# leggedrobotics/open3d_slam_private

Measured on AMD Instinct MI355X. Metric: ICP iterations/sec (scan-to-map), higher is better.
Workload: dtype f32

## Files before the change

### open3d_slam_private_amd/capi.py

```python
from __future__ import annotations

import ctypes as C
import math
import os
import subprocess

import numpy as np

_HERE = os.path.dirname(os.path.abspath(__file__))
_SO = os.environ.get("O3D_REG_LIB") or os.path.join(_HERE, "lib", "libo3dslam_reg.so")

STATUS_NAMES = {0: "OK", 1: "EMPTY_TARGET", 2: "EMPTY_SOURCE", 3: "NO_CORRESPONDENCES", 4: "BAD_TRANSFORM",
                5: "NOT_CONFIGURED", 6: "BAD_ARGUMENT", 7: "MISSING_FIELD", 8: "DEVICE_ERROR", 9: "UNSUPPORTED",
                10: "OUT_OF_BOUNDS"}
OUT_OF_BOUNDS = 10
COST_P2PL, COST_GICP = 0, 1
COST_O3D_P2PL, COST_O3D_P2P = 2, 3
SMOOTH_LEN_MAX = 15


class RegError(RuntimeError):
    def __init__(self, status, msg=""):
        self.status = status
        super().__init__(f"{STATUS_NAMES.get(status, status)}: {msg}")
# ... 1359 lines not shown
    lib = load_library()
    s = np.ascontiguousarray(sums, np.float64)
    To = np.zeros(16, np.float32)
    rank = C.c_int32()
    st = lib.reg_solve_update(C.byref(params), _ptr(s), _ptr(_T_in(T_iter)), _ptr(To), C.byref(rank))
    if st != 0:
        raise RegError(st, "reg_solve_update")
    return _T_out(To), rank.value


def host_solve6(A, b):
    x = np.zeros(6, np.float32)
    rank = load_library().reg_host_solve6(_ptr(_f32(A).reshape(36)), _ptr(_f32(b)), _ptr(x))
    return x, rank


def host_solve6_xicp(A, b, flags):
    x = np.zeros(6, np.float32)
    f = np.ascontiguousarray(flags, np.int32)
    rank = load_library().reg_host_solve6_xicp(_ptr(_f32(A).reshape(36)), _ptr(_f32(b)), _ptr(f), _ptr(x))
    return x, rank


def host_x_to_T(x):
    T = np.zeros(16, np.float32)
    load_library().reg_host_x_to_T(_ptr(_f32(x)), _ptr(T))
    return _T_out(T)


def host_centroid(xyz):
    xyz = _f32(xyz)
    out = np.zeros(3, np.float32)
    load_library().reg_host_centroid(_ptr(xyz), xyz.shape[1], xyz.shape[0], _ptr(out))
    return out


def host_o3d_update(cost, sums):
    s = np.ascontiguousarray(sums, np.float64).reshape(32)
    U = np.zeros(16, np.float64)
    rank = C.c_int32()
    st = load_library().reg_host_o3d_update(int(cost), _ptr(s), _ptr(U), C.byref(rank))
    if st != 0:
        raise RegError(st, "reg_host_o3d_update")
    return U.reshape(4, 4).T.copy(), rank.value


def host_tail_plan(n, cus=256, tile=0):
    lib = load_library()
    lib.reg_host_tail_plan.argtypes = [C.c_int64, C.c_int32, C.c_int32, C.POINTER(C.c_int32)]
    lib.reg_host_tail_plan.restype = None
    out = (C.c_int32 * 4)()
    lib.reg_host_tail_plan(int(n), int(cus), int(tile), out)
    return bool(out[0]), int(out[1]), int(out[2]), int(out[3])
```

### open3d_slam_private_amd/csrc/host_loop.hpp

```cpp
#pragma once


static reg_status check_ready(reg_handle* h, bool need_prepared) {
    if (!h) return REG_BAD_ARGUMENT;
    if (!h->device_ok) return REG_DEVICE_ERROR;
    if (h->m == 0) {
        h->err = "no reference set (reg_set_target)";
        return REG_NOT_CONFIGURED;
    }
    if (h->n == 0) {
        h->err = "no reading set (reg_set_source)";
        return REG_NOT_CONFIGURED;
    }
    if (need_prepared && !h->prepared) {
        h->err = "reg_prepare has not been called for this reading";
        return REG_NOT_CONFIGURED;
    }
    return REG_OK;
}

static reg_status prepare_rowmajor(reg_handle* h, const float* T_init_row, const float* c_override = nullptr,
                                   int64_t n_global = 0, const IterState* init_state = nullptr) {
    reg_status s = check_ready(h, false);
    if (s != REG_OK) return s;
// ... 44 lines not shown
        si.init = *init_state;
        si.dst = h->i_iter.as<IterState>();
    } else {
        std::memset(&si.init, 0, sizeof(si.init));
    }
    k_prepare_source<<<grid_for(n), 256, 0, h->stream>>>(
        h->s_raw.as<float>(), h->s_stride, (p2pl && h->has_snrm) ? h->s_nrm_raw.as<float>() : nullptr, h->s_nstride, n, pa,
        p2pl ? 1 : 0, h->perm, h->s_xyz.as<float4>(), (p2pl && h->has_snrm) ? h->s_nrm.as<float4>() : nullptr,
        h->i_hint.as<uint8_t>(), h->i_hist.as<uint32_t>(), h->i_acc.as<double>(), kAccRows * kSums, si,
        h->i_cache.as<float4>());
    if (h->prm.cost == REG_COST_GICP)
        k_pack_cov<<<grid_for(n), 256, 0, h->stream>>>(h->s_cov_raw.as<float>(), n, h->perm, h->s_cov.as<float4>());
    pmark("prepare_source");
    HIPCHK(h, hipGetLastError());
    h->prepared = true;
    h->match_launches = 0;
    h->have_match = false;
    h->pm_have_match = false;
    return REG_OK;
}


static void xicp_frame_change(const reg_handle* h, float Trd12[12]) {
    float A[16], Trd[16];
    m4_identity(A);
    for (int k = 0; k < 3; ++k) A[4 * k + 3] = -h->c_ref[k];
    m4_mul(A, h->T_init, Trd);
    for (int k = 0; k < 12; ++k) Trd12[k] = Trd[k];
}

static reg_status build_iter_state(reg_handle* h, const float* T_row, int update, IterState* st) {
    std::memset(st, 0, sizeof(IterState));
    for (int i = 0; i < 16; ++i) {
        st->T[i] = T_row[i];
        st->Td[i] = (double)T_row[i];
    }
    st->chk = Checkers();
    st->chk.max_iter = h->prm.max_iter;
    st->chk.min_diff_rot = h->prm.min_diff_rot;
    st->chk.min_diff_trans = h->prm.min_diff_trans;
    st->chk.smooth_len = h->prm.smooth_len;
    st->chk.init(T_row);
    st->cost = h->prm.cost;
    st->fixed_iters = h->prm.fixed_iters;
    st->max_iter = h->prm.max_iter;
    st->update = update;
    st->gicp_rot_eps = h->prm.gicp_rot_eps;
    st->gicp_trans_eps = h->prm.gicp_trans_eps;
    st->gicp_stop_rule = h->prm.gicp_stop_rule;
    st->gicp_rel_fitness = h->prm.gicp_rel_fitness;
    st->gicp_rel_rmse = h->prm.gicp_rel_rmse;
    st->n_total = (float)(h->n_total_hint > 0 ? h->n_total_hint : h->n);
    st->band_lo = st->band_hi = INFINITY;
    st->limit_last = st->limit_prev = INFINITY;
    st->use_trim = (h->prm.cost == REG_COST_P2PL && h->prm.use_trimmed) ? 1 : 0;
    st->trim_ratio = h->prm.trim_ratio;
    st->band_cap = kBandCap;
    st->qcount = h->i_qcount.as<unsigned int>();
    st->debug_narrow_band = ((h->dbg.debug_flags & 8) ? 1 : 0) | ((h->dbg.debug_flags & 64) ? 2 : 0);
    h->xicp_pending = false;
    for (int k = 0; k < 6; ++k) st->xicp_flags[k] = 1;
    if (h->prm.use_xicp && h->prm.cost == REG_COST_P2PL && update) {
        HIPCHK(h, h->i_xicp.reserve(sizeof(XicpState)));
        st->xicp_stage = 1;
        st->xicp_enough = h->prm.xicp_enough;
        st->xicp_insufficient = h->prm.xicp_insufficient;
        st->xicp_cos_min = (float)std::cos((double)h->prm.xicp_min_angle_deg * 3.14159265358979323846 / 180.0);
        st->xicp_cos_strong = (float)std::cos((double)h->prm.xicp_strong_angle_deg * 3.14159265358979323846 / 180.0);
        xicp_frame_change(h, st->xicp_Trd);
        h->xicp_pending = true;
    }
    return REG_OK;
}

static reg_status init_iter_state(reg_handle* h, const float* T_row, int update) {
    IterState* st = h->h_iter;
    if (h->iter_copy_pending) HIPCHK(h, hipEventSynchronize(h->ev_iter));
    reg_status s = build_iter_state(h, T_row, update, st);
    if (s != REG_OK) return s;
    HIPCHK(h, hipMemcpyAsync(h->i_iter.p, st, sizeof(IterState), hipMemcpyHostToDevice, h->stream));
    HIPCHK(h, hipEventRecord(h->ev_iter, h->stream));
    h->iter_copy_pending = true;
    return REG_OK;
}

static reg_status enqueue_match(reg_handle* h, bool zero_hist = false) {
    const bool trim = h->prm.cost == REG_COST_P2PL && h->prm.use_trimmed;
    if (trim && zero_hist) HIPCHK(h, hipMemsetAsync(h->i_hist.p, 0, 3 * 2048 * 4, h->stream));
    const bool fused_hist = h->dbg.match_variant == 3;
    uint32_t* hist0 = (trim && fused_hist) ? h->i_hist.as<uint32_t>() : nullptr;
    uint32_t* hist2 = trim ? h->i_hist.as<uint32_t>() + 4096 : nullptr;
    const IterState* it = h->i_iter.as<IterState>();
    if (h->dbg.match_variant == 1) {
        prof_mark(h, 0, true);
        k_match<<<h->n_blocks, 256, 0, h->stream>>>(h->s_xyz.as<float4>(), h->n, it, h->grid, h->i_pos.as<int>(),
                                                    h->i_d2.as<float>(), hist0, hist2, h->shift0);
        prof_mark(h, 0, false);
    } else {
        uint8_t* hint = h->dbg.match_variant == 2 ? nullptr : h->i_hint.as<uint8_t>();
        const int lanes = h->dbg.lanes_per_point == 4 ? 4 : (h->dbg.lanes_per_point == 2 ? 2 : 8);
        const int blocks = grid_for(h->n * lanes);
        const int tile = h->match_launches < 2 ? h->env.xcd_tile_first : h->env.xcd_tile_later;
        ++h->match_launches;
        const dim3 grid(xcd_tiled_grid(blocks, tile)), block(256);
        auto go = [&](auto kernel) {
            launch_timed(h, 0, kernel, grid, block, 0, (const float4*)h->s_xyz.as<float4>(), h->n, it, h->grid,
                         h->i_pos.as<int>(), h->i_d2.as<float>(), hist0, hist2, hint, h->shift0, h->dbg.debug_flags, blocks,
// ... 441 lines not shown
    if (h->env.hints) {
        std::vector<uint8_t> hv((size_t)h->n);
        if (hipMemcpy(hv.data(), h->i_hint.p, (size_t)h->n, hipMemcpyDeviceToHost) == hipSuccess) {
            long long cnt[18] = {0};
            for (uint8_t v : hv) ++cnt[v < 17 ? v : 17];
            fprintf(stderr, "[o3dreg] terminating level of the last iteration (halo, then levels with rho =");
            for (int l = 0; l < h->grid.n_levels; ++l) fprintf(stderr, " %.3f", h->grid.rho[l]);
            fprintf(stderr, "):");
            for (int l = 0; l <= h->grid.n_levels; ++l) fprintf(stderr, " %lld", cnt[l]);
            fprintf(stderr, "\n");
        }
    }
    if (h->env.coh_stats) {
        CohStats cs;
        if (hipMemcpy(&cs, h->i_stats.p, sizeof(cs), hipMemcpyDeviceToHost) == hipSuccess) {
            fprintf(stderr, "[o3dreg] coherent fused iterations: %llu point-iterations, %llu searched (%.2f %%)\n", cs.n_points,
                    cs.n_searched, cs.n_points ? 100.0 * (double)cs.n_searched / (double)cs.n_points : 0.0);
            (void)hipMemset(h->i_stats.p, 0, sizeof(cs));
        }
    }
    if (h->env.stamps) {
        fprintf(stderr, "update kernel stamps (cycles): reduce %llu [rows %llu select %llu band-add %llu] solve %llu update+check %llu mirror %llu\n", mir->stamps[0],
                mir->stamps[4], mir->stamps[5], mir->stamps[6], mir->stamps[1], mir->stamps[2], mir->stamps[3]);
        fprintf(stderr, "   select detail: verify+stage-issue %llu, zero+hist+barriers %llu, wave0 pick/rank %llu\n", mir->stamps[3], mir->stamps[7] >> 32, mir->stamps[7] & 0xffffffffull);
    }
    if (h->profiling) {
        for (size_t i = 0; i + 1 < h->prof_ev.size(); i += 2) {
            float ms = 0;
            if (hipEventElapsedTime(&ms, h->prof_ev[i], h->prof_ev[i + 1]) == hipSuccess) {
                const int kind = h->prof_kind[i / 2];
                res->prof_ms[kind] += ms;
                res->prof_launches[kind] += 1;
            }
        }
        for (hipEvent_t e : h->prof_ev) (void)hipEventDestroy(e);
        h->prof_ev.clear();
        h->prof_kind.clear();
        h->profiling = false;
    }
}

static reg_status register_pm(reg_handle* h, const float* Ti, float T_out[16], reg_result* res);

extern "C" {

void reg_host_tail_plan(int64_t n, int32_t cus, int32_t tile, int32_t plan[4]) {
    const TailPlan pl = tail_plan_for(n, cus, 0, tile);
    plan[0] = pl.ok ? 1 : 0;
    plan[1] = pl.grid;
    plan[2] = pl.wpc;
    plan[3] = pl.chunk8;
}

reg_status reg_prepare(reg_handle* h, const float T_init[16]) {
    if (!h || !T_init) return REG_BAD_ARGUMENT;
    float Tr[16];
    col_to_row(T_init, Tr);
    return prepare_rowmajor(h, Tr);
}

reg_status reg_linearize(reg_handle* h, const float T_iter[16], float H[36], float b[6], double* err,
                         int64_t* n_inliers) {
    reg_status s = check_ready(h, true);
    if (s != REG_OK) return s;
    if (!T_iter) return REG_BAD_ARGUMENT;
    if (h->prm.cost == REG_COST_O3D_P2P) {
        h->err = "reg_linearize: point-to-point (Umeyama) has no normal equations";
        return REG_UNSUPPORTED;
    }
    if (h->pm_on) {
        h->err = "reg_linearize: not available with a libpointmatcher chain (reg_set_pm_chain)";
        return REG_UNSUPPORTED;
    }
    float Tr[16];
    col_to_row(T_iter, Tr);
    if (!m4_is_finite(Tr)) return REG_BAD_TRANSFORM;
    HIPCHK(h, hipSetDevice(h->prm.device));
    s = iterate_once(h, Tr, true);
    if (s != REG_OK) return s;
    const double* sums = h->h_mirror->sums;
    if (H && b) sums_to_system(sums, h->prm.cost, H, b);
    if (err) *err = sums[27];
    if (n_inliers) *n_inliers = (int64_t)llround(sums[28]);
    if (sums[28] == 0.0) {
        h->err = "ErrorMinimizer: no point to minimize";
        return REG_NO_CORRESPONDENCES;
    }
    return REG_OK;
}

reg_status reg_register(reg_handle* h, const float T_init[16], float T_out[16], reg_result* res) {
    if (!h || !T_init || !T_out) return REG_BAD_ARGUMENT;
    reg_result local;
    if (!res) res = &local;
    std::memset(res, 0, sizeof(*res));
    std::memcpy(T_out, T_init, 64);
    float Ti[16];
    col_to_row(T_init, Ti);
    const auto t_reg0 = std::chrono::steady_clock::now();
    auto rmark = [&](const char* what) {
        if (h->env.trace)
            fprintf(stderr, "[o3dreg] register %-14s t=%.1fus\n", what,
                    std::chrono::duration<double, std::micro>(std::chrono::steady_clock::now() - t_reg0).count());
    };
    if (h->pm_on) return register_pm(h, Ti, T_out, res);
    const bool p2pl = h->prm.cost == REG_COST_P2PL;
// ... 199 lines not shown
```

### open3d_slam_private_amd/csrc/kernels_tail.hpp

```cpp
#pragma once

#ifndef O3D_TAIL_ACQ
#define O3D_TAIL_ACQ 0
#endif
#ifndef O3D_TAIL_THREADS
#define O3D_TAIL_THREADS 512
#endif
constexpr int kTailThreads = O3D_TAIL_THREADS;
#ifndef O3D_TAIL_SLOTS
#define O3D_TAIL_SLOTS 1024
#endif
#ifndef O3D_TAIL_WGS_PER_CU
#define O3D_TAIL_WGS_PER_CU 1
#endif
constexpr int kTailSlots = O3D_TAIL_SLOTS;
constexpr int kTailWgsPerCu = O3D_TAIL_WGS_PER_CU;
constexpr int kTailPts = kTailSlots / kTailThreads;
constexpr int kTailBandCap = 1024;
constexpr int kTailRec = 12;
constexpr int kTailHistRow = 32;
constexpr int kTailCoarse = 256;
constexpr float kTailWideRel = 0.02f;
constexpr int kTailMaxIters = 64;
constexpr int kTailSyncWords = 256;
constexpr int kTailRing = 4;
constexpr int kTailBandCntWord = 128;
constexpr int kTailAccRows = 16;
constexpr int kTailAccDoubles = kTailRing * kTailAccRows * kSums;
constexpr int kTailSyncBytes = kTailSyncWords * 4 + kTailAccDoubles * 8;
constexpr int kTailArriveStride = 16;
constexpr int kTailErrWord = 192;
constexpr int kTailSearchedWord = 193;
constexpr int kTailItersWord = 194;
constexpr int kTailCauseWord = 195;
constexpr int kTailStampWord = 200;
constexpr int kTailGroups = kTailThreads / 8;
constexpr int kTailBins = 1024;
#ifndef O3D_TAIL_STAMPS
#define O3D_TAIL_STAMPS 0
#endif
#ifndef O3D_TAIL_G4
#define O3D_TAIL_G4 0
#endif
#if O3D_TAIL_STAMPS
#define TAIL_STAMP(i)                                                      \
    do {                                                                   \
        const unsigned long long now_ = __builtin_amdgcn_s_memrealtime();  \
        stamp_acc[i] += now_ - stamp_last;                                 \
        stamp_last = now_;                                                 \
    } while (0)
#else
#define TAIL_STAMP(i) do { } while (0)
#endif

struct TailCfg {
    int64_t n;
    int chunk8;
    int wpc;
    int tile;
    int max_iters;
    float slack;
    unsigned long long seq;
    unsigned long long timeout_ticks;
};

struct TailLds {
    static constexpr int kRows = 0;
    static constexpr int kUnion = kRows + 5 * kTailSlots * 16;
    static constexpr int kUnionSeg = (kTailThreads / 8) * kSegWords<8> * 4, kUnionSeg4 = O3D_TAIL_G4 ? (kTailThreads / 4) * kSegWords<4> * 4 : 0;
    static constexpr int kUnionMax = kUnionSeg > kUnionSeg4 ? (kUnionSeg > kTailBandCap * 8 ? kUnionSeg : kTailBandCap * 8)
                                                            : (kUnionSeg4 > kTailBandCap * 8 ? kUnionSeg4 : kTailBandCap * 8);
    static constexpr int kUnionBytes = (kUnionMax + 255) & ~255;
    static constexpr int kD2 = kUnion + kUnionBytes;
    static constexpr int kFail = kD2 + kTailSlots * 4;
    static constexpr int kWcls = kFail + kTailSlots * 2;
    static constexpr int kHint = kWcls + kTailSlots;
    static constexpr int kSh = kHint + kTailSlots;
    static constexpr int kTot = kSh + 16 * kSums * 8;
    static constexpr int kState = kTot + kSums * 8;
    static constexpr int kStateBytes = (int)((sizeof(IterState) + 15) & ~size_t(15));
    static constexpr int kMisc = kState + kStateBytes;
    static constexpr int kWtot = kMisc + 64;
    static constexpr int kOff = kWtot + 64;
    static constexpr int kX = kOff + 272 * 4;
    static constexpr int kMirror = kX + 96;
    static constexpr int kMirrorBytes = (int)((sizeof(HostMirror) + 15) & ~size_t(15));
    static constexpr int kHist = kMirror + kMirrorBytes;
    static constexpr int kTotal = kHist + kTailBins * 4;
    static constexpr int kBk = kUnion;
};
static_assert(TailLds::kBk + kTailBandCap * 8 - TailLds::kUnion <= TailLds::kUnionBytes, "phase-C scratch exceeds the union");
static_assert(kTailGroups * kSegWords<8> * 4 <= TailLds::kUnionBytes, "segment lists exceed the union");
static_assert(TailLds::kTotal * kTailWgsPerCu <= 160 * 1024, "LDS budget of one CU");
constexpr int kTailLdsBytes = TailLds::kTotal;

__device__ __forceinline__ double tail_ld_f64(const double* p) {
    const unsigned long long v = __hip_atomic_load(reinterpret_cast<unsigned long long*>(const_cast<double*>(p)), __ATOMIC_RELAXED,
                                                   __HIP_MEMORY_SCOPE_AGENT);
    return __longlong_as_double((long long)v);
}
__device__ __forceinline__ void tail_st_f64(double* p, double x) {
    __hip_atomic_store(reinterpret_cast<unsigned long long*>(p), (unsigned long long)__double_as_longlong(x), __ATOMIC_RELAXED,
                       __HIP_MEMORY_SCOPE_AGENT);
}
__device__ __forceinline__ unsigned long long tail_ld_u64(const void* p) {
    return __hip_atomic_load(reinterpret_cast<unsigned long long*>(const_cast<void*>(p)), __ATOMIC_RELAXED, __HIP_MEMORY_SCOPE_AGENT);
}
__device__ __forceinline__ void tail_st_u64(void* p, unsigned long long x) {
    __hip_atomic_store(reinterpret_cast<unsigned long long*>(p), x, __ATOMIC_RELAXED, __HIP_MEMORY_SCOPE_AGENT);
}
__device__ __forceinline__ unsigned tail_ld_u32(const unsigned* p) {
    return __hip_atomic_load(const_cast<unsigned*>(p), __ATOMIC_RELAXED, __HIP_MEMORY_SCOPE_AGENT);
}

__device__ __noinline__ void tail_solve_update(IterState* sit, const double* tot, const uint32_t* misc, float* s_x, bool trim,
                                               unsigned n_band_raw) {
    const int lane = (int)(threadIdx.x & 63);
    const float r_limit_last = sit->limit_last, r_limit_sel = __uint_as_float(misc[2]);
    const int r_dbg_narrow = sit->debug_narrow_band & 1;
    const int r_fixed = sit->fixed_iters, r_iters = sit->iterations;
    const int r_xnc = sit->xicp_nc;
    const double r_tot28 = tot[28];
    float r_T[16];
#pragma unroll
    for (int i = 0; i < 16; ++i) r_T[i] = sit->T[i];
    const int r = lane >> 3, c = lane & 7;
    double a = 0.0;
    if (r < 6 && c < 7) {
        if (c < 6) {
            const int lo = r < c ? r : c, hi = r < c ? c : r;
            const int k = lo * 6 - (lo * (lo - 1)) / 2 + (hi - lo);
            a = (double)(float)tot[k];
        } else {
            a = (double)(-(float)tot[21 + r]);
        }
    }
    const double a_orig = a;
    double dmax = 0.0;
#pragma unroll
    for (int j = 0; j < 6; ++j) dmax = fmax(dmax, fabs(__shfl(a_orig, j * 8 + j)));
    bool well = dmax > 0.0;
    const double piv_thr = 1e-4 * dmax;
#pragma unroll
    for (int j = 0; j < 6; ++j) {
        const double pj = __shfl(a, j * 8 + j);
        well = well && (pj > piv_thr);
        const double ajc = __shfl(a, j * 8 + c);
        const double arj = __shfl(a, r * 8 + j);
        const double qd = ajc / pj;
        a = (r == j) ? qd : a - arj * qd;
    }
    double xsol[6];
#pragma unroll
    for (int i = 0; i < 6; ++i) xsol[i] = __shfl(a, i * 8 + 6);
    if (lane != 0) return;
    const float limit = r_limit_sel;
    sit->limit_prev = r_limit_last;
    sit->limit_last = limit;
    if (!trim || !(limit < INFINITY)) {
        sit->band_lo = INFINITY;
        sit->band_hi = INFINITY;
    } else {
        const float prev = r_limit_last;
        float m = 0.3f;
        if (prev < INFINITY && prev > 0.f) m = fminf(fmaxf(2.0f * fabsf(limit - prev) / limit + 0.003f, 0.003f), 0.6f);
        if (r_dbg_narrow) m = 1e-7f;
        sit->band_lo = limit * (1.0f - m);
        sit->band_hi = limit * (1.0f + m);
    }
    sit->band_count = n_band_raw;
    sit->stall = 0;
    if (r_tot28 == 0.0) {
        sit->status = REG_NO_CORRESPONDENCES;
        sit->done = 1;
        return;
    }
    float x[6], dT[16], Tn[16];
    int rank = 6;
    if (r_xnc > 0) {
        rank = upd_solve6_xicp(tot, sit->xicp_flags, s_x);
        for (int i = 0; i < 6; ++i) x[i] = s_x[i];
    } else if (well) {
        for (int i = 0; i < 6; ++i) x[i] = (float)xsol[i];
    } else {
        rank = upd_solve6_p2pl(tot, s_x);
        for (int i = 0; i < 6; ++i) x[i] = s_x[i];
    }
    sit->rank_last = rank;
    x_to_T(x, dT);
    m4_mul(dT, r_T, Tn);
    for (int i = 0; i < 16; ++i) sit->T_prev[i] = r_T[i];
    for (int i = 0; i < 16; ++i) sit->T[i] = Tn[i];
    sit->iterations = r_iters + 1;
    bool iterate;
    if (r_fixed > 0)
        iterate = r_iters + 1 < r_fixed;
    else
        iterate = sit->chk.check(Tn);
    if (!iterate) sit->done = 1;
}

__device__ __forceinline__ void tail_gicp_factor(const Xf& T, const float4 s, const float4 a0, const float4 a1, const float4 q,
                                                 const float4 b0, const float4 b1, float d2, double (&v)[kSums]) {
    const float3 tp = xf_point(T, s.x, s.y, s.z);
    const double r[3] = {(double)q.x - (double)tp.x, (double)q.y - (double)tp.y, (double)q.z - (double)tp.z};
    const double Cp[9] = {a0.x, a0.y, a0.z, a0.y, a0.w, a1.x, a0.z, a1.x, a1.y};
    const double Cq[9] = {b0.x, b0.y, b0.z, b0.y, b0.w, b1.x, b0.z, b1.x, b1.y};
    double R[9];
#pragma unroll
    for (int a = 0; a < 3; ++a)
#pragma unroll
        for (int c = 0; c < 3; ++c) R[3 * a + c] = (double)T.m[4 * a + c];
    double RC[9], S[9];
#pragma unroll
    for (int a = 0; a < 3; ++a)
#pragma unroll
        for (int c = 0; c < 3; ++c) {
            double t = 0;
#pragma unroll
            for (int k = 0; k < 3; ++k) t += R[3 * a + k] * Cp[3 * k + c];
            RC[3 * a + c] = t;
// ... 44 lines not shown
        }
        Mr[a] = Mi[3 * a] * r[0] + Mi[3 * a + 1] * r[1] + Mi[3 * a + 2] * r[2];
    }
    int k = 0;
#pragma unroll
    for (int a = 0; a < 6; ++a)
#pragma unroll
        for (int c = a; c < 6; ++c) {
            double t = 0;
#pragma unroll
            for (int kk = 0; kk < 3; ++kk) t += J[6 * kk + a] * MJ[6 * kk + c];
            v[k++] += t;
        }
#pragma unroll
    for (int a = 0; a < 6; ++a) v[21 + a] += J[a] * Mr[0] + J[6 + a] * Mr[1] + J[12 + a] * Mr[2];
    v[27] += 0.5 * (r[0] * Mr[0] + r[1] * Mr[1] + r[2] * Mr[2]);
    v[28] += 1.0;
    v[29] += 1.0;
    v[30] += (double)d2;
}

__device__ __noinline__ void tail_solve_update_gicp(IterState* sit, const double* tot, double* s_dl) {
    const int lane = (int)(threadIdx.x & 63);
    const int r = lane >> 3, c = lane & 7;
    double a = 0.0;
    if (r < 6 && c < 7) {
        if (c < 6) {
            const int lo = r < c ? r : c, hi = r < c ? c : r;
            a = tot[lo * 6 - (lo * (lo - 1)) / 2 + (hi - lo)];
        } else {
            a = -tot[21 + r];
        }
    }
    const double a_orig = a;
    double dmax = 0.0;
#pragma unroll
    for (int j = 0; j < 6; ++j) dmax = fmax(dmax, fabs(__shfl(a_orig, j * 8 + j)));
    bool well = dmax > 0.0;
    const double piv_thr = 1e-10 * dmax;
#pragma unroll
    for (int j = 0; j < 6; ++j) {
        const double pj = __shfl(a, j * 8 + j);
        well = well && (pj > piv_thr);
        const double ajc = __shfl(a, j * 8 + c);
        const double arj = __shfl(a, r * 8 + j);
        const double qd = ajc / pj;
        a = (r == j) ? qd : a - arj * qd;
    }
    double xsol[6];
#pragma unroll
    for (int i = 0; i < 6; ++i) xsol[i] = __shfl(a, i * 8 + 6);
    if (lane != 0) return;
    const double cnt = tot[28];
    sit->limit_prev = sit->limit_last;
    sit->limit_last = INFINITY;
    sit->band_lo = INFINITY;
    sit->band_hi = INFINITY;
    sit->band_count = 0;
    sit->stall = 0;
    float r_T[16];
    for (int i = 0; i < 16; ++i) r_T[i] = sit->T[i];
    if (cnt == 0.0) {
        sit->status = REG_NO_CORRESPONDENCES;
        sit->done = 1;
        return;
    }
    const double fit = cnt / (double)sit->n_total, rmse = sqrt(tot[30] / cnt);
    if (sit->gicp_stop_rule == 1 && sit->fixed_iters <= 0) {
        const bool conv = sit->iterations >= 1 && fabs(fit - sit->fit_prev) < (double)sit->gicp_rel_fitness &&
                          fabs(rmse - sit->rmse_prev) < (double)sit->gicp_rel_rmse;
        if (conv || sit->iterations >= sit->max_iter) {
            if (conv)
                sit->chk.converged = true;
            else
                sit->chk.max_iter_reached = true;
            for (int i = 0; i < 16; ++i) sit->T_prev[i] = r_T[i];
            sit->done = 1;
            return;
        }
    }
    sit->fit_prev = fit;
    sit->rmse_prev = rmse;
    double dl[6], E[16], Tn[16];
    int rank = 6;
    if (well) {
        for (int i = 0; i < 6; ++i) dl[i] = xsol[i];
    } else {
        rank = upd_solve_sym6(tot, s_dl);
        for (int i = 0; i < 6; ++i) dl[i] = s_dl[i];
    }
    sit->rank_last = rank;
    se3_exp(dl, E);
    for (int i = 0; i < 4; ++i)
        for (int j = 0; j < 4; ++j) {
            double v = 0;
            for (int kk = 0; kk < 4; ++kk) v += sit->Td[4 * i + kk] * E[4 * kk + j];
            Tn[4 * i + j] = v;
        }
    for (int i = 0; i < 16; ++i) {
        sit->T_prev[i] = r_T[i];
        sit->Td[i] = Tn[i];
        sit->T[i] = (float)Tn[i];
    }
    sit->iterations += 1;
    if (sit->fixed_iters > 0) {
        if (sit->iterations >= sit->fixed_iters) sit->done = 1;
// ... 236 lines not shown
            const int pprev = __float_as_int(tq.w);
            bool pass = false;
            const float attr_ok = kGicp ? st_rows[4 * kTailSlots + sl].w : nn.w;
            if (valid[u] && c.w > 0.f && pprev >= 0 && attr_ok == 1.f) {
                const float dx = p[u].x - tq.x, dy = p[u].y - tq.y, dz = p[u].z - tq.z;
                float a = dx * dx;
                float b2 = dy * dy;
                float d2 = a + b2;
                a = dz * dz;
                d2 = d2 + a;
                const float ex = p[u].x - c.x, ey = p[u].y - c.y, ez = p[u].z - c.z;
                const float delta = __builtin_amdgcn_sqrtf(ex * ex + ey * ey + ez * ez);
                const float lhs = (__builtin_amdgcn_sqrtf(d2) + delta) * 1.00001f + 1e-30f;
                const float rhs = __builtin_amdgcn_sqrtf(c.w) * 0.99999f;
                pass = d2 <= g.max_d2 && lhs < rhs;
                if (ru.w == 1.f) {
                    const float fx = p[u].x - ru.x, fy = p[u].y - ru.y, fz = p[u].z - ru.z;
                    float a2 = fx * fx;
                    float b3 = fy * fy;
                    float r2 = a2 + b3;
                    a2 = fz * fz;
                    r2 = r2 + a2;
                    pass = pass && d2 < r2;
                }
                if (pass) d2s[sl] = d2;
            }
            if (valid[u] && !pass) {
                const unsigned at = atomicAdd(&misc[0], 1u);
                fail[at] = (uint16_t)sl;
                st_rows[sl] = make_float4(p[u].x, p[u].y, p[u].z, -1.f);
            }
        }
        __syncthreads();
        TAIL_STAMP(0);
        const int nf = (int)misc[0];
        n_searched += (t == 0) ? (unsigned)nf : 0u;
        auto search_rounds = [&](auto gtag) {
            constexpr int G = decltype(gtag)::value;
            constexpr int kGroups = kTailThreads / G;
            const int sub = t & (G - 1), grp = t / G;
            for (int base = 0; base < nf; base += kGroups) {
                const int fi = base + grp;
                if (fi < nf) {
                    const int slot = (int)fail[fi];
                    const float4 a0 = st_rows[slot];
                    const float3 p2 = make_float3(a0.x, a0.y, a0.z);
                    const int hv = (int)hnt[slot];
                    int lvl;
                    float cov2;
                    const Best bb = nearest_group<G, O3D_COH_PRUNE != 0, true>(g, p2, sub, -1, &lvl, seg_lds + grp * kSegWords<G>,
                                                                               hv >= 2 ? hv - 2 : -1, &cov2, cfg.slack);
                    if (sub == 0) {
                        hnt[slot] = (uint8_t)(lvl + 1);
                        const int pc = bb.pos >= 0 ? bb.pos : 0;
                        float4 tq, nn;
                        if (kGicp) {
                            tq = g.pts[pc];
                            nn = tgt_nrm[2 * (size_t)pc];
                            float4 c1 = tgt_nrm[2 * (size_t)pc + 1];
                            c1.w = 1.f;
                            st_rows[4 * kTailSlots + slot] = c1;
                        } else {
                            tq = tgt_nrm[2 * (size_t)pc];
                            nn = tgt_nrm[2 * (size_t)pc + 1];
                            nn.w = 1.f;
                        }
                        float4 ru = make_float4(INFINITY, INFINITY, INFINITY, 1.f);
                        if (bb.pos2 >= 0) {
                            const float4 t2 = g.pts[bb.pos2];
                            ru = make_float4(t2.x, t2.y, t2.z, 1.f);
                        }
                        tq.w = __int_as_float(bb.pos);
                        st_rows[slot] = make_float4(p2.x, p2.y, p2.z, bb.pos >= 0 ? fminf(bb.third, cov2) : -1.f);
                        st_rows[kTailSlots + slot] = tq;
                        st_rows[2 * kTailSlots + slot] = nn;
                        st_rows[3 * kTailSlots + slot] = ru;
                        d2s[slot] = bb.pos >= 0 ? bb.d2 : INFINITY;
                    }
                }
            }
        };
#if O3D_TAIL_G4
        if (nf > kTailThreads / 8)
            search_rounds(std::integral_constant<int, 4>());
        else
#endif
            search_rounds(std::integral_constant<int, 8>());
        __syncthreads();
        TAIL_STAMP(1);
        float rF[kTailPts][7], md2v[kTailPts], wv[kTailPts];
        int clsv[kTailPts];
        const unsigned set = epoch & (kTailRing - 1);
        int buf = (int)(epoch & 1u);
        {
            double v[kSums];
#pragma unroll
            for (int k = 0; k < kSums; ++k) v[k] = 0.0;
#pragma unroll
            for (int u = 0; u < kTailPts; ++u) {
                const int sl = t + u * kTailThreads;
#pragma unroll
                for (int k = 0; k < 7; ++k) rF[u][k] = 0.f;
                const float4 tq = st_rows[kTailSlots + sl], nn = st_rows[2 * kTailSlots + sl];
                const int mpos = valid[u] ? __float_as_int(tq.w) : -1;
                const float md2 = d2s[sl];
                float w = 0.f;
                int cls = 2;
                if (kGicp) {
                    if (valid[u] && mpos >= 0) {
                        w = 1.f;
                        cls = 0;
                        tail_gicp_factor(T, s[u], sn[u], sc1[u], tq, nn, st_rows[4 * kTailSlots + sl], md2, v);
                    }
                } else if (valid[u] && mpos >= 0) {
                    w = 1.f;
                    if (f.use_maxdist && !(md2 <= f.outlier_max_d2)) w = 0.f;
                    if (f.use_normal) {
                        const float3 nr = normalize3(xf_rot(T, sn[u].x, sn[u].y, sn[u].z));
                        const float3 nt = normalize3(make_float3(nn.x, nn.y, nn.z));
                        float a = nr.x * nt.x;
                        float bb2 = nr.y * nt.y;
                        float val = a + bb2;
                        a = nr.z * nt.z;
                        val = val + a;
                        if (val < f.cos_max_angle) w = 0.f;
                    }
                    cls = md2 < band_lo ? 0 : (md2 < band_hi ? 1 : 2);
                    if (w != 0.f && cls != 2) {
                        float a = p[u].y * nn.z, bq = p[u].z * nn.y;
                        rF[u][0] = a - bq;
                        a = p[u].z * nn.x; bq = p[u].x * nn.z;
                        rF[u][1] = a - bq;
                        a = p[u].x * nn.y; bq = p[u].y * nn.x;
                        rF[u][2] = a - bq;
                        rF[u][3] = nn.x; rF[u][4] = nn.y; rF[u][5] = nn.z;
                        const float dx = p[u].x - tq.x, dy = p[u].y - tq.y, dz = p[u].z - tq.z;
                        float r = dx * nn.x;
                        float t2 = dy * nn.y;
                        r = r + t2;
                        t2 = dz * nn.z;
// ... 225 lines not shown
                }
                __syncthreads();
                TAIL_STAMP(8);
#pragma unroll
                for (int u = 0; u < kTailPts; ++u)
                    if (my_bin[u] == misc[6]) bk[atomicAdd(&misc[9], 1u)] = ((unsigned long long)my_u[u] << 32) | (unsigned)(t + u * kTailThreads);
                __syncthreads();
                {
                    const uint32_t csel = misc[8], rsel = misc[7];
                    for (uint32_t i = (uint32_t)t; i < csel; i += kTailThreads) {
                        const unsigned long long e = bk[i];
                        uint32_t rr = 0;
                        for (uint32_t j = 0; j < csel; ++j) rr += bk[j] < e ? 1u : 0u;
                        if (rr == rsel) misc[2] = (uint32_t)(e >> 32);
                    }
                }
                __syncthreads();
                TAIL_STAMP(9);
                const float limit = __uint_as_float(misc[2]);
                double v[kSums];
#pragma unroll
                for (int k = 0; k < kSums; ++k) v[k] = 0.0;
#pragma unroll
                for (int u = 0; u < kTailPts; ++u) {
                    const unsigned i = (unsigned)(t + u * kTailThreads);
                    const unsigned long long* r6 = u == 0 ? rv : rv2;
                    const float d2r = __uint_as_float((unsigned)(r6[3] >> 32)), keptr = __uint_as_float((unsigned)r6[4]);
                    if (i < n_band && d2r <= limit && keptr != 0.f) {
                        const float F[7] = {__uint_as_float((unsigned)r6[0]), __uint_as_float((unsigned)(r6[0] >> 32)),
                                            __uint_as_float((unsigned)r6[1]), __uint_as_float((unsigned)(r6[1] >> 32)),
                                            __uint_as_float((unsigned)r6[2]), __uint_as_float((unsigned)(r6[2] >> 32)),
                                            __uint_as_float((unsigned)r6[3])};
                        accumulate(v, F, d2r);
                    }
                }
                wave_reduce32(v);
                if ((lane & 1) == 0) sh[wave][lane >> 1] = v[0];
                __syncthreads();
                if (t < kSums) {
                    double v2 = 0.0;
#pragma unroll
                    for (int w2 = 0; w2 < kWaves; ++w2) v2 += sh[w2][t];
                    tot[t] += v2;
                }
                __syncthreads();
            }
        }
        TAIL_STAMP(10);
        if (t < kSums) sit->sums[t] = tot[t];
        if (wave == 0) {
            if (kGicp)
                tail_solve_update_gicp(sit, tot, reinterpret_cast<double*>(s_x));
            else
                tail_solve_update(sit, tot, misc, s_x, trim, n_band_raw);
        }
        __syncthreads();
        TAIL_STAMP(11);
        if (sit->done) {
            exit_reason = 1;
            ++k_local;
            break;
        }
        if (k_local + 1 >= cfg.max_iters) {
            exit_reason = 3;
            ++k_local;
            break;
        }
    }
    if (exit_reason == 2 || exit_reason == 4) {
        if (t == 0) {
            sit->stall = 1;
            sit->band_count = 0;
        }
        __syncthreads();
    }
#pragma unroll
    for (int u = 0; u < kTailPts; ++u) {
        if (!valid[u]) continue;
        const int sl = t + u * kTailThreads;
        const float4 tq = st_rows[kTailSlots + sl];
        const int cls = (int)(wcls[sl] >> 1);
        float w = (wcls[sl] & 1) ? 1.f : 0.f;
        if (cls == 1 && !(d2s[sl] <= __uint_as_float(misc[2]))) w = 0.f;
        pos_io[q[u]] = __float_as_int(tq.w);
        d2_out[q[u]] = d2s[sl];
        if (w_out) w_out[q[u]] = w;
        if (hint_g) hint_g[q[u]] = hnt[sl];
    }
    if (exit_reason == 3) {
        for (int sl = t; sl < kTailSlots; sl += kTailThreads) {
            const int64_t oc = (int64_t)(sl >> 3) * cfg.wpc + wq;
            const int64_t r_in = oc * 8 + (sl & 7);
            int64_t qq;
            if (cfg.tile > 0) {
                const int64_t tl = oc / cfg.tile, rr = oc - tl * cfg.tile;
                qq = ((tl * 8 + xcls) * cfg.tile + rr) * 8 + (sl & 7);
            } else {
                qq = (int64_t)xcls * cfg.chunk8 + r_in;
            }
            if (r_in < cfg.chunk8 && qq < n) {
#pragma unroll
                for (int r = 0; r < 4; ++r) cache[(size_t)r * (size_t)n + qq] = st_rows[r * kTailSlots + sl];
            }
        }
    }
    if (t == 0 && n_searched) atomicAdd(&sync[kTailSearchedWord], n_searched);
#if O3D_TAIL_STAMPS
// ... 62 lines not shown
```

### open3d_slam_private_amd/csrc/kernels_update.hpp

```cpp
#pragma once

__global__ void __launch_bounds__(64)
k_pack_contrib(double* __restrict__ acc, const IterState* __restrict__ it, float* __restrict__ contrib) {
    const int c = threadIdx.x;
    double* hdr = reinterpret_cast<double*>(contrib);
    if (it->done || it->stall) {
        if (c < kSums) hdr[c] = 0.0;
        if (c == 0) reinterpret_cast<uint32_t*>(contrib)[64] = 0u;
        return;
    }
    if (c < kSums) {
        double t = 0;
        for (int r = 0; r < kAccRows; ++r) {
            t += acc[(size_t)r * kSums + c];
            acc[(size_t)r * kSums + c] = 0.0;
        }
        hdr[c] = t;
    }
    if (c == 0) reinterpret_cast<uint32_t*>(contrib)[64] = it->band_count;
}

__device__ __forceinline__ void lds_barrier() {
    asm volatile("s_waitcnt lgkmcnt(0)" ::: "memory");
    __builtin_amdgcn_s_barrier();
// ... 388 lines not shown
        __syncthreads();
    }
    if (threadIdx.x < kSums) sit->sums[threadIdx.x] = tot[threadIdx.x];
    if (threadIdx.x >= 64 && threadIdx.x < 64 + kQueues && sit->qcount) sit->qcount[(threadIdx.x - 64) * kQueueStride] = 0u;
    if (threadIdx.x >= 64) return;
    const int lane = threadIdx.x;
    const unsigned long long st1 = __builtin_amdgcn_s_memtime();
    unsigned long long st2 = st1, st3 = st1;
    const bool p2pl = !kO3d && sit->cost == REG_COST_P2PL;
    const float r_limit_last = sit->limit_last, r_limit_sel = s_limit;
    const int r_dbg_narrow = sit->debug_narrow_band & 1, r_update = sit->update, r_xstage = sit->xicp_stage;
    const int r_fixed = sit->fixed_iters, r_iters = sit->iterations;
    int r_xnc = sit->xicp_nc;
    const unsigned r_band_count = sit->band_count;
    const double r_tot28 = tot[28];
    float r_T[16];
#pragma unroll
    for (int i = 0; i < 16; ++i) r_T[i] = sit->T[i];
    const int r = lane >> 3, c = lane & 7;
    double a = 0.0;
    if (r < 6 && c < 7) {
        if (c < 6) {
            const int lo = r < c ? r : c, hi = r < c ? c : r;
            const int k = lo * 6 - (lo * (lo - 1)) / 2 + (hi - lo);
            a = p2pl ? (double)(float)tot[k] : tot[k];
        } else {
            a = p2pl ? (double)(-(float)tot[21 + r]) : -tot[21 + r];
        }
    }
    const double a_orig = a;
    double dmax = 0.0;
#pragma unroll
    for (int j = 0; j < 6; ++j) dmax = fmax(dmax, fabs(__shfl(a_orig, j * 8 + j)));
    bool well = dmax > 0.0;
    const double piv_thr = (p2pl ? 1e-4 : 1e-10) * dmax;
#pragma unroll
    for (int j = 0; j < 6; ++j) {
        const double pj = __shfl(a, j * 8 + j);
        well = well && (pj > piv_thr);
        const double ajc = __shfl(a, j * 8 + c);
        const double arj = __shfl(a, r * 8 + j);
        const double q = ajc / pj;
        a = (r == j) ? q : a - arj * q;
    }
    double xsol[6];
#pragma unroll
    for (int i = 0; i < 6; ++i) xsol[i] = __shfl(a, i * 8 + 6);
    st2 = __builtin_amdgcn_s_memtime();
    const bool stage_a = !finish && r_update != 0 && p2pl && r_xstage == 1 && r_tot28 != 0.0 && xs != nullptr;
    if (stage_a && lane < 2) upd_xicp_stage_a(tot, sit->xicp_Trd, lane == 0 ? xs->vr : xs->vt, lane == 0 ? 0 : 3);
    if (lane == 0) {
        const float limit = finish ? r_limit_last : r_limit_sel;
        if (!finish) {
            sit->limit_prev = r_limit_last;
            sit->limit_last = limit;
        }
        if (finish) {
        } else if (!trim || !(limit < INFINITY)) {
            sit->band_lo = INFINITY;
            sit->band_hi = INFINITY;
        } else {
            const float prev = r_limit_last;
            float m = 0.3f;
            if (prev < INFINITY && prev > 0.f) m = fminf(fmaxf(2.0f * fabsf(limit - prev) / limit + 0.003f, 0.003f), 0.6f);
            if (r_dbg_narrow) m = 1e-7f;
            sit->band_lo = limit * (1.0f - m);
            sit->band_hi = limit * (1.0f + m);
        }
        const int nband_report = (int)r_band_count;
        sit->band_count = 0;
        sit->stall = 0;
        bool do_update = r_update != 0;
        if (stage_a) {
            for (int i = 0; i < 4; ++i) xs->center[i] = 0.0;
            for (int i = 0; i < 6; ++i) {
                xs->comb[i] = 0.0;
                xs->high[i] = 0.0;
            }
            sit->xicp_stage = 2;
            do_update = false;
            s_skip_mirror = 1;
        }
        if (finish && xs) {
            int nc = 0;
            for (int i = 0; i < 6; ++i) {
                const int ok = (xs->comb[i] >= (double)sit->xicp_enough || xs->high[i] >= (double)sit->xicp_insufficient) ? 1 : 0;
                sit->xicp_flags[i] = ok;
                sit->xicp_comb[i] = xs->comb[i];
                sit->xicp_high[i] = xs->high[i];
                nc += ok ? 0 : 1;
            }
            sit->xicp_nc = nc;
            r_xnc = nc;
            sit->xicp_stage = 0;
        }
        if (do_update) {
            if (r_tot28 == 0.0) {
                sit->status = REG_NO_CORRESPONDENCES;
                sit->done = 1;
            } else if (p2pl) {
                float x[6], dT[16], Tn[16];
                int rank = 6;
                if (r_xnc > 0) {
                    rank = upd_solve6_xicp(tot, sit->xicp_flags, s_x);
                    for (int i = 0; i < 6; ++i) x[i] = s_x[i];
                } else if (well) {
                    for (int i = 0; i < 6; ++i) x[i] = (float)xsol[i];
                } else {
                    rank = upd_solve6_p2pl(tot, s_x);
                    for (int i = 0; i < 6; ++i) x[i] = s_x[i];
                }
                sit->rank_last = rank;
                x_to_T(x, dT);
                m4_mul(dT, r_T, Tn);
                for (int i = 0; i < 16; ++i) sit->T_prev[i] = r_T[i];
                for (int i = 0; i < 16; ++i) sit->T[i] = Tn[i];
                sit->iterations = r_iters + 1;
                bool iterate;
                if (r_fixed > 0)
                    iterate = r_iters + 1 < r_fixed;
// ... 202 lines not shown
```

### open3d_slam_private_amd/csrc/reg_state.hpp

```cpp
#pragma once

struct IterState {
    float T[16];
    float T_prev[16];
    double Td[16];
    Checkers chk;
    int iterations;
    int done;
    int status;
    int rank_last;
    int cost;
    int fixed_iters;
    int max_iter;
    int update;
    float gicp_rot_eps, gicp_trans_eps;
    int gicp_stop_rule;
    float gicp_rel_fitness, gicp_rel_rmse;
    float n_total;
    double fit_prev, rmse_prev;
    double sums[kSums];
    float band_lo, band_hi;
    float trim_ratio;
    int use_trim;
    int stall;
    float limit_last;
    float limit_prev;
    unsigned int band_count;
    unsigned int* qcount;
    unsigned int band_cap;
    int debug_narrow_band;
    int xicp_stage;
    int xicp_nc;
    int xicp_flags[6];
    float xicp_enough, xicp_insufficient, xicp_cos_min, xicp_cos_strong;
    float xicp_Trd[12];
    double xicp_comb[6], xicp_high[6];
};

struct XicpState {
    float vr[9], vt[9];
    int pad[2];
    double center[4];
    double comb[6], high[6];
};

struct HostMirror {
    double sums[kSums];
    float T[16];
    float T_prev[16];
    int iterations, done, status, rank_last, converged, max_iter_reached, stall, band_count;
    float limit_last, limit_prev, band_lo, band_hi;
    int pad_nband, pad2;
    int localizable[6];
    int n_constraints, pad3;
    double xicp_comb[6], xicp_high[6];
    unsigned long long stamps[8];
    unsigned long long seq;
    struct SeqRecord {
        unsigned long long seq;
        int iterations, done, stall, pad;
        float limit_last, limit_prev;
    } ring[16];
};
constexpr int kSeqRing = 16;
constexpr int kQueues = 64;
constexpr int kQueueStride = 16;

__device__ __forceinline__ int xcd_block(int n_blocks) {
    const int chunk = (n_blocks + 7) >> 3;
    return (int)(blockIdx.x & 7) * chunk + (int)(blockIdx.x >> 3);
}

__host__ __device__ __forceinline__ int xcd_tiled_grid(int n_blocks, int tile) {
    if (tile <= 0) return 8 * ((n_blocks + 7) / 8);
    const int per = 8 * tile;
    return per * ((n_blocks + per - 1) / per);
}
__device__ __forceinline__ int xcd_block_tiled(int n_blocks, int tile) {
    if (tile <= 0) return xcd_block(n_blocks);
    const int xcd = (int)(blockIdx.x & 7), j = (int)(blockIdx.x >> 3);
    const int t = j / tile, r = j - t * tile;
    return (t * 8 + xcd) * tile + r;
}

struct Xf4 {
    float m[16];
};

__device__ __forceinline__ Xf load_xf(const IterState* it) {
    Xf x;
#pragma unroll
    for (int k = 0; k < 12; ++k) x.m[k] = it->T[k];
    return x;
}
```

Before: 16960.

## Predict trim band from limit trend and defer correspondence row gathers

```diff
diff --git a/open3d_slam_private_amd/capi.py b/open3d_slam_private_amd/capi.py
--- a/open3d_slam_private_amd/capi.py
+++ b/open3d_slam_private_amd/capi.py
@@ -1435,3 +1435,25 @@
     out = (C.c_int32 * 4)()
     lib.reg_host_tail_plan(int(n), int(cus), int(tile), out)
     return bool(out[0]), int(out[1]), int(out[2]), int(out[3])
+
+
+def host_predict_band(limit, prev=math.inf, prev2=math.inf, last_count=0, last_lo=math.inf, last_hi=math.inf, debug_narrow=0):
+    lib = load_library()
+    lib.reg_host_predict_band.argtypes = [C.c_float, C.c_float, C.c_float, C.c_uint32, C.c_float, C.c_float, C.c_int32,
+                                          C.POINTER(C.c_float), C.POINTER(C.c_float)]
+    lib.reg_host_predict_band.restype = None
+    out = (C.c_float * 2)()
+    lib.reg_host_predict_band(float(limit), float(prev), float(prev2), int(last_count), float(last_lo), float(last_hi),
+                              int(debug_narrow), out, None)
+    return np.float32(out[0]), np.float32(out[1])
+
+
+def host_band_constants():
+    lib = load_library()
+    lib.reg_host_predict_band.argtypes = [C.c_float, C.c_float, C.c_float, C.c_uint32, C.c_float, C.c_float, C.c_int32,
+                                          C.POINTER(C.c_float), C.POINTER(C.c_float)]
+    lib.reg_host_predict_band.restype = None
+    c = (C.c_float * 8)()
+    lib.reg_host_predict_band(math.inf, math.inf, math.inf, 0, math.inf, math.inf, 0, None, c)
+    names = ("band_cap", "wide_rel", "floor", "ratio_max", "centre_gain", "geom_rel", "guard_frac", "forced_wide")
+    return {k: float(np.float32(v)) for k, v in zip(names, c)}
diff --git a/open3d_slam_private_amd/csrc/host_loop.hpp b/open3d_slam_private_amd/csrc/host_loop.hpp
--- a/open3d_slam_private_amd/csrc/host_loop.hpp
+++ b/open3d_slam_private_amd/csrc/host_loop.hpp
@@ -120,7 +120,7 @@
     st->gicp_rel_rmse = h->prm.gicp_rel_rmse;
     st->n_total = (float)(h->n_total_hint > 0 ? h->n_total_hint : h->n);
     st->band_lo = st->band_hi = INFINITY;
-    st->limit_last = st->limit_prev = INFINITY;
+    st->limit_last = st->limit_prev = st->limit_prev2 = INFINITY;
     st->use_trim = (h->prm.cost == REG_COST_P2PL && h->prm.use_trimmed) ? 1 : 0;
     st->trim_ratio = h->prm.trim_ratio;
     st->band_cap = kBandCap;
@@ -668,6 +668,20 @@
     plan[3] = pl.chunk8;
 }
 
+REG_API void reg_host_predict_band(float limit, float prev, float prev2, uint32_t last_count, float last_lo, float last_hi,
+                                   int32_t debug_narrow, float band[2], float consts[8]) {
+    const Band b = predict_band(limit, prev, prev2, last_count, last_lo, last_hi, debug_narrow);
+    if (band) {
+        band[0] = b.lo;
+        band[1] = b.hi;
+    }
+    if (consts) {
+        const float c[8] = {(float)kTailBandCap, kTailWideRel, kBandFloor, kBandRatioMax, kBandCentreGain, kBandGeomRel, kBandGuardFrac,
+                            kBandForcedWide};
+        for (int i = 0; i < 8; ++i) consts[i] = c[i];
+    }
+}
+
 reg_status reg_prepare(reg_handle* h, const float T_init[16]) {
     if (!h || !T_init) return REG_BAD_ARGUMENT;
     float Tr[16];
diff --git a/open3d_slam_private_amd/csrc/kernels_tail.hpp b/open3d_slam_private_amd/csrc/kernels_tail.hpp
--- a/open3d_slam_private_amd/csrc/kernels_tail.hpp
+++ b/open3d_slam_private_amd/csrc/kernels_tail.hpp
@@ -16,11 +16,9 @@
 constexpr int kTailSlots = O3D_TAIL_SLOTS;
 constexpr int kTailWgsPerCu = O3D_TAIL_WGS_PER_CU;
 constexpr int kTailPts = kTailSlots / kTailThreads;
-constexpr int kTailBandCap = 1024;
 constexpr int kTailRec = 12;
 constexpr int kTailHistRow = 32;
 constexpr int kTailCoarse = 256;
-constexpr float kTailWideRel = 0.02f;
 constexpr int kTailMaxIters = 64;
 constexpr int kTailSyncWords = 256;
 constexpr int kTailRing = 4;
@@ -114,7 +112,7 @@
 }
 
 __device__ __noinline__ void tail_solve_update(IterState* sit, const double* tot, const uint32_t* misc, float* s_x, bool trim,
-                                               unsigned n_band_raw) {
+                                               unsigned n_band_raw, unsigned n_band_all) {
     const int lane = (int)(threadIdx.x & 63);
     const float r_limit_last = sit->limit_last, r_limit_sel = __uint_as_float(misc[2]);
     const int r_dbg_narrow = sit->debug_narrow_band & 1;
@@ -155,18 +153,15 @@
     for (int i = 0; i < 6; ++i) xsol[i] = __shfl(a, i * 8 + 6);
     if (lane != 0) return;
     const float limit = r_limit_sel;
+    const float r_limit_prev = sit->limit_prev;
+    sit->limit_prev2 = r_limit_prev;
     sit->limit_prev = r_limit_last;
     sit->limit_last = limit;
-    if (!trim || !(limit < INFINITY)) {
-        sit->band_lo = INFINITY;
-        sit->band_hi = INFINITY;
-    } else {
-        const float prev = r_limit_last;
-        float m = 0.3f;
-        if (prev < INFINITY && prev > 0.f) m = fminf(fmaxf(2.0f * fabsf(limit - prev) / limit + 0.003f, 0.003f), 0.6f);
-        if (r_dbg_narrow) m = 1e-7f;
-        sit->band_lo = limit * (1.0f - m);
-        sit->band_hi = limit * (1.0f + m);
+    {
+        const Band nb = trim ? predict_band(limit, r_limit_last, r_limit_prev, n_band_all, sit->band_lo, sit->band_hi, r_dbg_narrow)
+                             : Band{INFINITY, INFINITY};
+        sit->band_lo = nb.lo;
+        sit->band_hi = nb.hi;
     }
     sit->band_count = n_band_raw;
     sit->stall = 0;
@@ -317,6 +312,7 @@
     for (int i = 0; i < 6; ++i) xsol[i] = __shfl(a, i * 8 + 6);
     if (lane != 0) return;
     const double cnt = tot[28];
+    sit->limit_prev2 = sit->limit_prev;
     sit->limit_prev = sit->limit_last;
     sit->limit_last = INFINITY;
     sit->band_lo = INFINITY;
@@ -659,29 +655,9 @@
                                                                                hv >= 2 ? hv - 2 : -1, &cov2, cfg.slack);
                     if (sub == 0) {
                         hnt[slot] = (uint8_t)(lvl + 1);
-                        const int pc = bb.pos >= 0 ? bb.pos : 0;
-                        float4 tq, nn;
-                        if (kGicp) {
-                            tq = g.pts[pc];
-                            nn = tgt_nrm[2 * (size_t)pc];
-                            float4 c1 = tgt_nrm[2 * (size_t)pc + 1];
-                            c1.w = 1.f;
-                            st_rows[4 * kTailSlots + slot] = c1;
-                        } else {
-                            tq = tgt_nrm[2 * (size_t)pc];
-                            nn = tgt_nrm[2 * (size_t)pc + 1];
-                            nn.w = 1.f;
-                        }
-                        float4 ru = make_float4(INFINITY, INFINITY, INFINITY, 1.f);
-                        if (bb.pos2 >= 0) {
-                            const float4 t2 = g.pts[bb.pos2];
-                            ru = make_float4(t2.x, t2.y, t2.z, 1.f);
-                        }
-                        tq.w = __int_as_float(bb.pos);
                         st_rows[slot] = make_float4(p2.x, p2.y, p2.z, bb.pos >= 0 ? fminf(bb.third, cov2) : -1.f);
-                        st_rows[kTailSlots + slot] = tq;
-                        st_rows[2 * kTailSlots + slot] = nn;
-                        st_rows[3 * kTailSlots + slot] = ru;
+                        st_rows[kTailSlots + slot].w = __int_as_float(bb.pos);
+                        st_rows[3 * kTailSlots + slot].w = __int_as_float(bb.pos2);
                         d2s[slot] = bb.pos >= 0 ? bb.d2 : INFINITY;
                     }
                 }
@@ -693,6 +669,28 @@
         else
 #endif
             search_rounds(std::integral_constant<int, 8>());
+        __syncthreads();
+#pragma unroll 1
+        for (int fi = tv; fi < nf; fi += kTailThreads) {
+            const int slot = (int)fail[fi];
+            const int pos = __float_as_int(st_rows[kTailSlots + slot].w), pos2 = __float_as_int(st_rows[3 * kTailSlots + slot].w);
+            const size_t pc = (size_t)(pos >= 0 ? pos : 0), pc2 = (size_t)(pos2 >= 0 ? pos2 : 0);
+            const float4 t2 = g.pts[pc2];
+            float4 tq = kGicp ? g.pts[pc] : tgt_nrm[2 * pc];
+            float4 nn = kGicp ? tgt_nrm[2 * pc] : tgt_nrm[2 * pc + 1];
+            if (kGicp) {
+                float4 c1 = tgt_nrm[2 * pc + 1];
+                c1.w = 1.f;
+                st_rows[4 * kTailSlots + slot] = c1;
+            } else {
+                nn.w = 1.f;
+            }
+            tq.w = __int_as_float(pos);
+            st_rows[kTailSlots + slot] = tq;
+            st_rows[2 * kTailSlots + slot] = nn;
+            st_rows[3 * kTailSlots + slot] = pos2 >= 0 ? make_float4(t2.x, t2.y, t2.z, 1.f)
+                                                       : make_float4(INFINITY, INFINITY, INFINITY, 1.f);
+        }
         __syncthreads();
         TAIL_STAMP(1);
         float rF[kTailPts][7], md2v[kTailPts], wv[kTailPts];
@@ -1024,7 +1022,7 @@
             if (kGicp)
                 tail_solve_update_gicp(sit, tot, reinterpret_cast<double*>(s_x));
             else
-                tail_solve_update(sit, tot, misc, s_x, trim, n_band_raw);
+                tail_solve_update(sit, tot, misc, s_x, trim, n_band_raw, wide ? misc[12] : n_band_raw);
         }
         __syncthreads();
         TAIL_STAMP(11);
diff --git a/open3d_slam_private_amd/csrc/kernels_update.hpp b/open3d_slam_private_amd/csrc/kernels_update.hpp
--- a/open3d_slam_private_amd/csrc/kernels_update.hpp
+++ b/open3d_slam_private_amd/csrc/kernels_update.hpp
@@ -464,20 +464,14 @@
     if (lane == 0) {
         const float limit = finish ? r_limit_last : r_limit_sel;
         if (!finish) {
+            const float r_limit_prev = sit->limit_prev;
+            sit->limit_prev2 = r_limit_prev;
             sit->limit_prev = r_limit_last;
             sit->limit_last = limit;
-        }
-        if (finish) {
-        } else if (!trim || !(limit < INFINITY)) {
-            sit->band_lo = INFINITY;
-            sit->band_hi = INFINITY;
-        } else {
-            const float prev = r_limit_last;
-            float m = 0.3f;
-            if (prev < INFINITY && prev > 0.f) m = fminf(fmaxf(2.0f * fabsf(limit - prev) / limit + 0.003f, 0.003f), 0.6f);
-            if (r_dbg_narrow) m = 1e-7f;
-            sit->band_lo = limit * (1.0f - m);
-            sit->band_hi = limit * (1.0f + m);
+            const Band nb = trim ? predict_band(limit, r_limit_last, r_limit_prev, n_band, sit->band_lo, sit->band_hi, r_dbg_narrow)
+                                 : Band{INFINITY, INFINITY};
+            sit->band_lo = nb.lo;
+            sit->band_hi = nb.hi;
         }
         const int nband_report = (int)r_band_count;
         sit->band_count = 0;
diff --git a/open3d_slam_private_amd/csrc/reg_state.hpp b/open3d_slam_private_amd/csrc/reg_state.hpp
--- a/open3d_slam_private_amd/csrc/reg_state.hpp
+++ b/open3d_slam_private_amd/csrc/reg_state.hpp
@@ -29,6 +29,7 @@
     unsigned int* qcount;
     unsigned int band_cap;
     int debug_narrow_band;
+    float limit_prev2;
     int xicp_stage;
     int xicp_nc;
     int xicp_flags[6];
@@ -63,6 +64,49 @@
     } ring[16];
 };
 constexpr int kSeqRing = 16;
+
+constexpr int kTailBandCap = 1024;
+constexpr float kTailWideRel = 0.02f;
+constexpr float kBandFloor = 0.003f;
+constexpr float kBandRatioMax = 0.6f;
+constexpr float kBandCentreGain = 1.5f;
+constexpr float kBandGeomRel = 0.25f;
+constexpr float kBandGuardFrac = 0.75f;
+constexpr float kBandForcedWide = 0.0205f;
+struct Band {
+    float lo, hi;
+};
+__host__ __device__ inline Band predict_band(float limit, float prev, float prev2, unsigned last_count, float last_lo, float last_hi,
+                                             int debug_narrow) {
+    Band b = {INFINITY, INFINITY};
+    if (!(limit < INFINITY)) return b;
+    float m = 0.3f;
+    if (prev < INFINITY && prev > 0.f) m = fminf(fmaxf(2.0f * fabsf(limit - prev) / limit + kBandFloor, kBandFloor), 0.6f);
+    if (debug_narrow) m = 1e-7f;
+    b.lo = limit * (1.0f - m);
+    b.hi = limit * (1.0f + m);
+    if (debug_narrow) return b;
+    if (prev < INFINITY && prev > 0.f && prev2 < INFINITY && prev2 > 0.f) {
+        const float d = limit - prev, dp = prev - prev2;
+        if (d * dp > 0.f && fabsf(d) < fabsf(dp) && fabsf(dp) <= kBandGeomRel * limit) {
+            const float q = d / dp;
+            const float far_edge = limit + fmaxf(kBandCentreGain * q, kBandRatioMax) * d, pad = kBandFloor * limit;
+            b.lo = d < 0.f ? far_edge - pad : limit - pad;
+            b.hi = d < 0.f ? limit + pad : far_edge + pad;
+        }
+    }
+    if (last_count > 0u && last_hi < INFINITY && last_hi > last_lo) {
+        const float est = (float)last_count * (b.hi - b.lo) / (last_hi - last_lo);
+        if (est > kBandGuardFrac * (float)kTailBandCap && !(b.hi - b.lo > kTailWideRel * b.lo)) {
+            const float grow = 0.5f * (kBandForcedWide * limit - (b.hi - b.lo));
+            if (grow > 0.f) {
+                b.lo -= grow;
+                b.hi += grow;
+            }
+        }
+    }
+    return b;
+}
 constexpr int kQueues = 64;
 constexpr int kQueueStride = 16;
 
```

Result: faster. 17730 (median of 6 runs) (+4.5%).
